# nanoporetech/bonito

Measured on AMD Instinct MI355X. Metric: signal samples/sec/GPU (chunk=10000, batch=512) + read accuracy vs ref, higher is better.
Workload: dtype f16

## Files before the change

bonito_amd/_lib.py:

```python
import ctypes as C
import os

_HERE = os.path.dirname(os.path.abspath(__file__))
LIB_PATH = os.environ.get("BONITO_HIP_LIB") or os.path.join(_HERE, "libbonito_hip.so")


class HipEngineError(RuntimeError):
    """An entry point of libbonito_hip.so reported an error."""


class bh_layer_t(C.Structure):
    _fields_ = [
        ("kind", C.c_int32), ("in_size", C.c_int32), ("out_size", C.c_int32),
        ("winlen", C.c_int32), ("stride", C.c_int32), ("padding", C.c_int32),
        ("activation", C.c_int32), ("reverse", C.c_int32),
        ("nhead", C.c_int32), ("dim_ff", C.c_int32), ("win_left", C.c_int32), ("win_right", C.c_int32),
        ("scale_factor", C.c_int32), ("groups", C.c_int32), ("add_residual", C.c_int32), ("quantize", C.c_int32), ("reserved_i", C.c_int32 * 1),
        ("scale", C.c_float), ("clamp_lo", C.c_float), ("clamp_hi", C.c_float),
        ("blank_score", C.c_float), ("alpha", C.c_float), ("eps", C.c_float), ("reserved_f", C.c_float * 2),
        ("w0", C.c_void_p), ("b0", C.c_void_p), ("w1", C.c_void_p), ("b1", C.c_void_p),
        ("w2", C.c_void_p), ("w3", C.c_void_p), ("w4", C.c_void_p), ("w5", C.c_void_p),
    ]


# ... 118 lines not shown
    "bh_host_map_finish": (_l, [_vp, _l, _vp, _l, _l, _vp, _l, _l, _vp, _l, _vp, _l, _vp, _l, _vp]),
    "bh_host_mean_qscore": (C.c_double, [C.c_char_p, _l]),
    "bh_host_svb16_decode": (_l, [_vp, _l, _l, _vp]),
    "bh_lstm_workspace": (_sz, [_i, _i]),
    "bh_lstm_layer": (_i, [_vp, _vp, _vp, _i, _i, _i, _i, _vp, _vp, _i, _vp]),
    "bh_lstm_q8_layer": (_i, [_vp, _f, _vp, _vp, _vp, _i, _i, _i, _i, _i, _vp, _vp, _vp, _vp]),
    "bh_lstm_q8_layer_split": (_i, [_vp, _f, _vp, _vp, _vp, _i, _i, _i, _i, _i, _vp, _vp, _vp, _i, _vp]),
    "bh_lstm_layer_family": (_i, [_vp, _vp, _vp, _vp, _i, _i, _i, _i, _i, _i, _vp, _vp]),
    "bh_lstm_launch_plan": (_i, [_i, _i, _i, _i, _i, C.POINTER(C.c_int32), _i]),
    "bh_optim_chunk": (_i, []),
    "bh_optim_workspace": (_sz, [_vp, _i]),
    "bh_optim_norm": (_i, [_vp, _vp, _i, _vp, _d, _i, _d, _d, _i, _d, _d, _vp, _sz, _vp]),
    "bh_optim_update": (_i, [_vp, _vp, _vp, _vp, _vp, _i, _vp, _d, _d, _d, _d, _d, _vp]),
    "bh_optim_last_kernel": (_i, []),
    "bh_encoder_debug_read": (_i, [_vp, _vp, _sz, _sz]),
    "bh_encoder_set_option": (_i, [_vp, C.c_char_p, _i]),
}

_lib = None


CONV_KERNELS = {"none": 0, "first": 1, "ws_384": 20, "ws_96": 21, "front3_384": 30, "front3_96": 31, "dwconv": 40, "igemm_base": 100}


def conv_igemm_code(ntt, fs):
    return CONV_KERNELS["igemm_base"] + 10 * ntt + int(fs)


CTC_LOSS_KERNELS = {1: 31, 2: 63, 4: 127, 8: 255, 104: 511, 108: 1023, 116: 2047}

# ... 44 lines not shown
```

bonito_amd/csrc/beam.hip:

```cpp
#include <stdlib.h>

#include "common.h"
#include "kernels.h"
#include "options.h"
#include <cstring>
#include "../../include/bh_lse_table.h"

namespace bh {

__device__ const float g_lse_tab[BH_LSE_TABLE_SIZE] = {BH_LSE_TABLE_VALUES};

__device__ __forceinline__ float lse2_tab(float a, float b, const float* tab) {
    float m = fmaxf(a, b);
    float d = fabsf(a - b);
    if (!(d < BH_LSE_RANGE)) return m;
    float x = d * BH_LSE_SCALE;
    int i = (int)x;
    float f = x - (float)i;
    float t0 = tab[i];
    float sp = __fmaf_rn(f, tab[i + 1] - t0, t0);
    return m + sp;
}

__device__ __forceinline__ float lse2_tab_nb(float a, float b, const float* tab) {
// ... 1126 lines not shown
    }
    if (DBG && lane == 0)
        for (int i = 0; i < 6; ++i) p.dbg[(long)n * 8 + i] = dsec[i];
}

struct FinArgs {
    const uint8_t* bp;
    const int* final_slot;
    const float* P;
    int N, T;
    float q_scale, q_offset;
    int8_t* sequence;
    int8_t* qstring;
    int8_t* moves;
    float* qfloat;
};

constexpr int FTB = 256;

__global__ __launch_bounds__(64) void beam_finalize_kernel(FinArgs p) {
    __shared__ __attribute__((aligned(16))) uint8_t st[FTB * MAXW];
    __shared__ int8_t res_m[FTB], res_s[FTB];
    __shared__ int s_r;
    const int n = blockIdx.x, lane = threadIdx.x;
    const int T = p.T;
    const uint8_t* bp = p.bp + (long)n * T * MAXW;
    const float* P = p.P + (long)n * T * 4;
    int8_t* sq = p.sequence + (long)n * T;
    int8_t* qs = p.qstring + (long)n * T;
    int8_t* mv = p.moves + (long)n * T;
    float* qf = p.qfloat ? p.qfloat + (long)n * T : nullptr;
    if (lane == 0) s_r = p.final_slot[n];
    for (int thi = T; thi > 0; thi -= FTB) {
        const int tlo = max(0, thi - FTB);
        const int nbytes = (thi - tlo) * MAXW;
        const uint4_t* src = (const uint4_t*)(bp + (long)tlo * MAXW);
        {
            constexpr int PER = FTB * MAXW / 16 / 64;
            uint4_t tmp[PER];
#pragma unroll
            for (int k = 0; k < PER; ++k)
                if (lane + 64 * k < nbytes / 16) tmp[k] = src[lane + 64 * k];
#pragma unroll
            for (int k = 0; k < PER; ++k)
                if (lane + 64 * k < nbytes / 16) ((uint4_t*)st)[lane + 64 * k] = tmp[k];
        }
        __syncthreads();
        if (lane == 0) {
            int r = s_r;
            for (int t = thi - 1; t >= tlo; --t) {
                const int info = st[(t - tlo) * MAXW + r];
                const int is_move = (info >> 5) & 1;
                res_m[t - tlo] = (int8_t)is_move;
                res_s[t - tlo] = is_move ? (int8_t)((0x54474341u >> (8 * (info >> 6))) & 0xffu) : (int8_t)0;
                r = info & 31;
            }
            s_r = r;
        }
        __syncthreads();
        for (int i = lane; i < thi - tlo; i += 64) {
            mv[tlo + i] = res_m[i];
            sq[tlo + i] = res_s[i];
            qs[tlo + i] = 0;
// ... 10 lines not shown
        const int c = sq[t];
        const int x = c == 'A' ? 0 : c == 'C' ? 1 : c == 'G' ? 2 : 3;
        double err = 0.0;
        for (int u = t; u < t2; ++u) {
            const float4_t pv = *(const float4_t*)(P + (long)u * 4);
#pragma unroll
            for (int y = 0; y < 4; ++y)
                if (y != x) err += (double)pv[y];
        }
        err /= (double)(t2 - t);
        if (err < 1e-10) err = 1e-10;
        float qv = (float)(-10.0 * log10(err)) * p.q_scale + p.q_offset;
        qv = fminf(fmaxf(qv, 1.0f), 50.0f);
        if (qf) qf[t] = qv;
        qs[t] = (int8_t)(33 + (int)floorf(qv + 0.5f));
    }
}

}

namespace {
using namespace bh;

size_t n_states(int state_len) {
    size_t S = 1;
    for (int i = 0; i < state_len; ++i) S *= 4;
    return S;
}

struct DecodeWorkspace {
// ... 183 lines not shown
    if (int rc = launch_instance(bs2_backward_instances, p.backward, stream, a2)) return rc;
    SideStream* side = p.forward_on_helper ? side_stream() : nullptr;
    if (side) {
        BH_CHECK_HIP(hipEventRecord(side->fork, stream));
        BH_CHECK_HIP(hipStreamWaitEvent(side->stream, side->fork, 0));
    }
    if (p.has_forward) {
        Bs2FwdArgs f2{(const half_t*)scores, beta, P, N, T, blank, p.nt};
        if (int rc = launch_instance(bs2_forward_instances, p.forward, side ? side->stream : stream, f2)) return rc;
    }
    if (side) BH_CHECK_HIP(hipEventRecord(side->join, side->stream));
    BeamArgs ba{(const half_t*)scores, beta, N, T, (int)n_states(state_len), state_len, beam_width, blank, logf(beam_cut), bp, fin,
                debug ? (long long*)(ws + w.dbg) : nullptr, p.select_radix ? 0.0f : 256.0f / fmaxf(logf(beam_cut), 1e-6f), P, p.nt};
    if (int rc = launch_instance(beam_instances, p.beam, stream, ba)) return rc;
    if (side) BH_CHECK_HIP(hipStreamWaitEvent(stream, side->join, 0));
    FinArgs fa{bp, fin, P, N, T, q_scale, q_offset, sequence, qstring, moves, qfloat};
    hipLaunchKernelGGL(beam_finalize_kernel, dim3(N), dim3(64), 0, stream, fa);
    BH_CHECK_HIP(hipGetLastError());
    return 0;
}

int bh_k_beam_search_plan(int N, int T, int state_len, int cu_count, int debug, int32_t* out, int n_out) {
    BH_REQUIRE(state_len >= 1 && state_len <= 5, "beam_search_plan: state_len must be in 1..5 (got %d)", state_len);
    BH_REQUIRE(N > 0 && T > 0 && out, "beam_search_plan: empty problem N=%d T=%d, or no record", N, T);
    const BeamPlan p = beam_plan(state_len, N, bh::g_opt, debug != 0, cu_count);
    const DecodeWorkspace w = decode_workspace(N, T, state_len);
    const int32_t plan[] = {bs2_backward_instances[p.backward.instance].key, p.backward.grid, p.backward.block, p.backward.lds,
                            p.has_forward, p.has_forward ? bs2_forward_instances[p.forward.instance].key : 0, p.forward.grid,
                            p.forward.block, p.forward.lds, p.forward_on_helper,
                            state_len, p.cpw, p.debug, p.fuse, p.beam.grid, p.beam.block, p.beam.lds, p.select_radix, p.nt};
    const size_t layout[] = {w.beta, w.Bcum, w.logZ, w.P, w.bp, w.fin, w.dbg, w.pv_bp, w.beam_total, w.pv_total};
    constexpr int n_plan = sizeof(plan) / sizeof(plan[0]), n_layout = sizeof(layout) / sizeof(layout[0]);
// ... 11 lines not shown
```

bonito_amd/csrc/engine.cpp:

```cpp
#include <hip/hip_runtime.h>
#include <stdarg.h>
#include <stdio.h>
#include <string.h>

#include <algorithm>
#include <atomic>
#include <cmath>
#include <string>
#include <vector>

#include "../../include/bonito_hip.h"
#include "common.h"
#include "devbuf.h"
#include "kernels.h"
#include "lstm_pack.h"
#include "options.h"

static thread_local char g_err[1024] = "";
void bh_set_error(const char* fmt, ...) {
    va_list ap;
    va_start(ap, fmt);
    vsnprintf(g_err, sizeof(g_err), fmt, ap);
    va_end(ap);
}
// ... 79 lines not shown
    std::vector<Layer> layers;
    DevBuf act[3], gates, sig, err, lstm_ws;
    static constexpr int ERR_SLOTS = 64;
    int* err_host = nullptr;
    std::atomic<long> ticket{-1};
    std::atomic<long> checked{-1};
    std::atomic<int> sticky{0};
    int* cur_err = nullptr;
    int n_act = 2;
    hipStream_t fill_stream = nullptr;
    hipEvent_t fill_ready = nullptr, fill_done = nullptr;
    void* prefilled = nullptr;
    int lstm_prefill = 1;
    DevBuf q_act[2], q_ex;
    DevBuf ex16;
    int lstm_pair = 1;
    int norm_fuse = 0;
    int lstm_exchange = 1;
    int lstm_q8 = 1;
    DevBuf res;
    DevBuf t_qkv, t_mid, t_a, t_b, rot;
    int rot_len = 0;
    int out_features = 0;
    int lstm_force_slow = 0, lstm_tune = 0;
    int batch_pad = 16;
    int lstm_wide = 1;
    int attn_ring = 1;
    int lstm_fused = 3;
    bool profiling = false;
    struct Span { int cls; hipEvent_t a, b; };
// ... 144 lines not shown
    if (!q8) {
        p.row = lstm_admits(d, p.family, wide && !ring ? BH_LSTM_V_OUTPUT : 0);
        p.geo = p.row->geo;
        p.handoff = p.geo.unlimited ? HANDOFF_LDS : p.row->ex_bytes ? HANDOFF_RING : HANDOFF_OUTPUT;
        if (!p.row->projects) {
            p.gate_w = l.lstm_ih[p.row->w_ih].p;
            p.gate_b = (const float*)(p.row->w_ih == BH_LSTM_W_WIDE_ROWS ? l.lstm_bias_wide : l.b0).p;
        }
    }
    p.n_rings = Np / p.geo.ring_chunks;
    p.rings_per_launch = p.geo.rings_per_launch(e->n_cus);
    p.pairs = p.family == BH_LSTM_WGX && e->lstm_pair;
    return p;
}

struct CreateState {
    int channels = 1, channels_eff = 1;
    float bound = 4.0f;
    bool any_q8 = false;
};

static int create_conv(bh_encoder* e, size_t i, const bh_layer_t& d, CreateState& cs) {
    Layer& L = e->layers[i];
    BH_REQUIRE(d.w0 && d.in_size > 0 && d.out_size > 0 && d.winlen > 0 && d.stride > 0, "encoder_create: layer %zu: malformed convolution", i);
    BH_REQUIRE(d.groups <= 1, "encoder_create: layer %zu: grouped conv not supported here", i);
    const bool next_is_conv = next_kind(e, i) == BH_LAYER_CONV;
    const int K = d.winlen;
    L.cin_eff = d.in_size == 1 ? 1 : cs.channels_eff;
    L.cout_eff = next_is_conv ? pad8(d.out_size) : d.out_size;
    BH_REQUIRE(d.in_size == 1 || (cs.channels == d.in_size && L.cin_eff >= d.in_size),
// ... 196 lines not shown
            bh_set_error("encoder_create: sentinel pre-fill resources");
            return -1;
        }
    }
    if (cs.any_q8) {
        if (e->q_act[0].alloc(ab + 256) || e->q_act[1].alloc(ab + 256) || e->q_ex.alloc((size_t)4 * (Np / 16) * 16 * 1024 + 256))
            return -1;
    }
    {
        size_t exb = 0;
        for (const auto& l : e->layers) {
            if (l.d.kind != BH_LAYER_LSTM) continue;
            for (const bh_lstm_instance* row : lstm_admitted(l.d)) exb = std::max(exb, (size_t)4 * (Np / row->geo.ring_chunks) * row->ex_bytes);
        }
        if (exb && e->ex16.alloc(exb + 256)) return -1;
    }
    if (e->act[0].alloc(ab + 256) || e->act[1].alloc(ab + 256) || e->gates.alloc(w.gate_bytes + 256) ||
        e->sig.alloc((size_t)Np * e->max_chunk * 2) || e->err.alloc(sizeof(int) * bh_encoder::ERR_SLOTS) ||
        e->lstm_ws.alloc(bh_k_lstm_ws_bytes(Np, 1024)))
        return -1;
    if (w.qkv_bytes) {
        if (e->t_qkv.alloc(w.qkv_bytes + 256) || e->t_mid.alloc(w.mid_bytes + 256) || e->t_a.alloc(w.model_bytes + 256) ||
            e->t_b.alloc(w.model_bytes + 256))
            return -1;
        std::vector<float> cs_table((size_t)w.max_tokens * 32 * 2);
        if (bh_rotary_table(w.max_tokens, 64, cs_table.data())) return -2;
        if (upload_f32(e->rot, cs_table.data(), cs_table.size())) return -1;
        e->rot_len = w.max_tokens;
    }
    if (hipHostMalloc((void**)&e->err_host, sizeof(int) * bh_encoder::ERR_SLOTS, hipHostMallocDefault) != hipSuccess) {
// ... 300 lines not shown
        }
    }
    e->prefilled = nullptr;
    if (next_kind(e, i) == BH_LAYER_LSTM) { rc = prefill_next(e, c, i, (size_t)M); if (rc) return rc; }
    ProfSpan span(e, st, BH_PROF_LSTM_REC);
    bh_lstm_launch layer{};
    layer.family = p.family;
    layer.input = p.gate_w ? e->gates.p : c.cur;
    layer.w_ih = l.lstm_ih[p.row->w_ih].p; layer.w_hh = l.lstm_hh[p.row->w_hh].p; layer.bias = (const float*)l.b0.p;
    layer.h_out = dst;
    layer.ex = p.handoff == HANDOFF_RING ? e->ex16.p : nullptr;
    layer.T = len; layer.N = Np; layer.H = H;
    layer.R = layer.n_rings = p.n_rings;
    layer.reverse = d.reverse;
    layer.err_flag = e->cur_err; layer.xcc_ws = (int*)e->lstm_ws.p;
    layer.write_through = e->lstm_force_slow; layer.tune = e->lstm_tune;
    rc = bh_k_lstm_run_layer(layer, p.rings_per_launch, p.pairs, st);
    if (rc) return rc;
    c.advance(dst); c.C = H;
    return 0;
}

static int forward_linear_crf(bh_encoder* e, size_t i, Cursor& c) {
    const Layer& l = e->layers[i];
    const bh_layer_t& d = l.d;
    BH_REQUIRE(c.lay == L_TNC || c.lay == L_NLC, "encoder_forward: linearcrfencoder needs encoded input");
    BH_REQUIRE(c.C == d.in_size, "encoder_forward: layer %zu expects %d features, got %d", i, d.in_size, c.C);
    const float sc = d.scale != 0.0f ? d.scale : 1.0f;
    int rc;
    ProfSpan span(e, c.st, BH_PROF_CRF_LINEAR);
// ... 144 lines not shown
    if (prev != e->device) BH_CHECK_HIP(hipSetDevice(e->device));
    struct Restore {
        int prev, dev;
        ~Restore() { if (prev != dev) (void)hipSetDevice(prev); }
    } restore{prev, e->device};

    {
        const long n = ++e->ticket;
        const int slot = (int)(n % bh_encoder::ERR_SLOTS);
        if (n - bh_encoder::ERR_SLOTS > e->checked.load()) e->sticky.fetch_or(((volatile int*)e->err_host)[slot]);
        ((volatile int*)e->err_host)[slot] = 0;
        e->cur_err = (int*)e->err.p + slot;
        BH_CHECK_HIP(hipMemsetAsync(e->cur_err, 0, sizeof(int), st));
    }
    const int Np = (N + e->batch_pad - 1) / e->batch_pad * e->batch_pad;
    if (Np != N) BH_CHECK_HIP(hipMemsetAsync((char*)e->sig.p + (size_t)N * L * 2, 0, (size_t)(Np - N) * L * 2, st));
    BH_CHECK_HIP(hipMemcpyAsync(e->sig.p, signal, (size_t)N * L * 2, hipMemcpyDeviceToDevice, st));

    e->prefilled = nullptr;
    Cursor c;
    c.cur = e->sig.p; c.len = L; c.N = N; c.Np = Np; c.st = st; c.scores = scores; c.n_act = e->n_act;
    for (size_t i = 0; i < e->layers.size(); ++i) {
        int rc = 0;
        switch (e->layers[i].d.kind) {
            case BH_LAYER_CLAMP: continue;
            case BH_LAYER_CONV: rc = forward_conv(e, i, c); break;
            case BH_LAYER_LSTM: rc = forward_lstm(e, i, c); break;
            case BH_LAYER_LINEAR_CRF: rc = forward_linear_crf(e, i, c); break;
            case BH_LAYER_LINEAR: rc = forward_linear(e, i, c); break;
            case BH_LAYER_TRANSFORMER: rc = forward_transformer(e, i, c); break;
            case BH_LAYER_DWCONV: rc = forward_dwconv(e, i, c); break;
            case BH_LAYER_RESIDUAL_PROJ: rc = forward_residual_proj(e, i, c); break;
            case BH_LAYER_CTC_DECODER: rc = forward_ctc_decoder(e, i, c); break;
            case BH_LAYER_UPSAMPLE: rc = forward_upsample(e, i, c); break;
            default: BH_REQUIRE(false, "encoder_forward: unsupported layer kind %d", e->layers[i].d.kind);
        }
// ... 69 lines not shown
        BH_CHECK_HIP(hipEventSynchronize(s.b));
        float t = 0.0f;
        BH_CHECK_HIP(hipEventElapsedTime(&t, s.a, s.b));
        if (s.cls >= 0 && s.cls < BH_PROF_CLASSES) { ms[s.cls] += t; launches[s.cls] += 1; }
        (void)hipEventDestroy(s.a); (void)hipEventDestroy(s.b);
    }
    e->spans.clear();
    return 0;
}

extern "C" int bh_encoder_debug_read(bh_encoder_t* e, void* host, size_t bytes, size_t offset) {
    BH_REQUIRE(e && host && offset + bytes <= e->lstm_ws.bytes, "encoder_debug_read: out of range");
    BH_CHECK_HIP(hipMemcpy(host, (char*)e->lstm_ws.p + offset, bytes, hipMemcpyDeviceToHost));
    return 0;
}
extern "C" int bh_encoder_set_option(bh_encoder_t* e, const char* name, int value) {
    BH_REQUIRE(e && name, "encoder_set_option: null argument");
    if (!strcmp(name, "lstm_force_slow")) { e->lstm_force_slow = value & 1; return 0; }
    if (!strcmp(name, "lstm_fused")) { e->lstm_fused = value; return 0; }
    if (!strcmp(name, "attn_ring")) { e->attn_ring = value; return 0; }
    if (!strcmp(name, "lstm_wide")) { e->lstm_wide = value; return 0; }
    if (!strcmp(name, "lstm_prefill")) { e->lstm_prefill = value; return 0; }
    if (!strcmp(name, "lstm_q8")) { e->lstm_q8 = value; return 0; }
    if (!strcmp(name, "lstm_exchange")) { e->lstm_exchange = value; return 0; }
    if (!strcmp(name, "lstm_pair")) { e->lstm_pair = value; return 0; }
    if (!strcmp(name, "norm_fuse")) { e->norm_fuse = value; return 0; }
    if (!strcmp(name, "gemm_v1")) { bh::g_opt.gemm_path = value; return 0; }
    if (!strcmp(name, "lstm_tune")) { e->lstm_tune = value; return 0; }
    BH_REQUIRE(false, "encoder_set_option: unknown option '%s'", name);
}
// ... 1 lines not shown
```

bonito_amd/csrc/kernels.h:

```cpp
#pragma once
#include <hip/hip_runtime.h>
#include <stdint.h>

#include "../../include/bonito_hip.h"

int bh_k_linear(const void* X, const void* W, const float* bias, void* out, int M, int N, int K,
                int ldx, int ldw, int ldo, int act, float scale, float clamp_lo, float clamp_hi,
                int gated, int row_div, long row_s_hi, long row_s_lo, int row_lim, hipStream_t stream,
                const void* residual = nullptr, int ldres = 0, float res_scale = 1.0f);
int bh_k_linear_last_kernel();

int bh_k_conv_first(const void* signal, const float* w, const float* bias, void* out, int N, int Lin,
                    int Lout, int Cout, int K, int stride, int pad, int act, float clamp_lo,
                    float clamp_hi, long os_n, long os_t, hipStream_t stream);
int bh_k_conv_igemm(const void* in, const void* wpk, const float* bias, void* out, int N, int Lin,
                    int Lout, int Cin, int Cout, int K, int stride, int pad, int act, float clamp_lo,
                    float clamp_hi, long os_n, long os_t, hipStream_t stream);
int bh_k_conv_last_kernel();
void bh_k_conv_note_kernel(int code);

struct bh_lstm_geometry {
    int ring_chunks = 16;
    int wgs_per_group = 0;
    int rings_per_slot = 1;
// ... 42 lines not shown
    bh_lstm_family family;
    const void* input;
    const void* w_ih;
    const void* w_hh;
    const float* bias;
    void* h_out;
    void* ex;
    int T, N, H;
    int R, n_rings;
    int reverse;
    int* err_flag;
    int* xcc_ws;
    int write_through;
    int tune;
    int arm;
};
int bh_k_lstm_launch(const bh_lstm_launch& l, hipStream_t stream);
int bh_k_lstm_run_layer(const bh_lstm_launch& layer, int rings_per_launch, bool pair, hipStream_t stream);
int bh_k_lstm_launch_plan(int family, int H, int flags, int n_rings, int cus, int32_t* out, int n_out);
size_t bh_k_lstm_ws_bytes(int N, int H);
int bh_k_fill_u16(void* dst, uint16_t value, size_t count, hipStream_t stream);

int bh_k_crf_viterbi(const void* scores, int N, int T, int state_len, int layout_5s, float blank_score,
                     long s_n, long s_t, void* bp_ws, float* alpha_ws, int8_t* moves, int8_t* path,
                     float* best_score, hipStream_t stream);

int bh_k_crf_revcomp(const void* in, void* out, int N, int T, int state_len, int layout_5s, long s_n, long s_t,
                     hipStream_t stream);

size_t bh_k_crf_seq_workspace(int N, int T, int Lmax, int state_len);
// ... 173 lines not shown
```

bonito_amd/csrc/lstm.hip:

```cpp
#include <string.h>
#include <type_traits>

#include "common.h"
#include "kernels.h"
#include "lstm_cell.h"
#include "lstm_ring.h"
#include "options.h"

namespace bh {

struct LstmArgs {
    const half_t* G;
    const half_t* whh;
    half_t* h;
    int T, N, H;
    int n_rings;
    int reverse;
    int* err;
    unsigned max_spins;
    int* xcc_ws;
    int force_slow;
    int tune;
};

// ... 1222 lines not shown
    p->grid = g.grid(n_rings);
    p->xcc_bytes = 0;
    p->arm_bytes = arm ? (size_t)4 * R * row->ex_bytes : 0;
    if (g.unlimited) return 0;
    BH_REQUIRE(g.wgs_per_group > 0 && p->grid <= g.resident(cus), "lstm: %d workgroups must be co-resident but the device has %d CUs; split the batch", p->grid, cus);
    p->xcc_bytes = (size_t)n_rings * row->slots_per_ring * sizeof(int);
    return 0;
}

int bh_k_lstm_launch(const bh_lstm_launch& l, hipStream_t stream) {
    using namespace bh;
    LstmLaunchPlan p;
    if (int rc = lstm_launch_plan(l.family, l.H, l.ex != nullptr, l.tune, l.N, l.R, l.n_rings, l.arm != 0, bh_cu_count(), &p)) return rc;
    const bh_lstm_instance& row = *p.row;
    BH_REQUIRE(!row.projects || l.input != l.h_out, "lstm: fused layer cannot run in place");
    if (!row.geo.unlimited) {
        BH_REQUIRE(l.xcc_ws != nullptr, "lstm: missing XCD agreement workspace");
        BH_CHECK_HIP(hipMemsetAsync(l.xcc_ws, 0xFF, p.xcc_bytes, stream));
    }
    if (p.arm_bytes) BH_CHECK_HIP(hipMemsetAsync(l.ex, 0xFF, p.arm_bytes, stream));
    const LstmArgs a{row.projects || row.args == ARGS_WIDE ? nullptr : (const half_t*)l.input, (const half_t*)l.w_hh, (half_t*)l.h_out,
                     l.T, l.N, l.H, l.n_rings, l.reverse, l.err_flag, max_spins(), l.xcc_ws, l.write_through, l.tune};
    const LstmFusedArgs fa{(const half_t*)l.input, (const half_t*)l.w_ih, l.bias, a};
    if (row.raise_lds) BH_CHECK_HIP(bh_max_lds(row.kernel, row.lds_bytes));
    const dim3 grid(p.grid), block(row.block);
    switch (row.args) {
        case ARGS_LSTM: hipLaunchKernelGGL(((void (*)(LstmArgs))row.kernel), grid, block, row.lds_bytes, stream, a); break;
        case ARGS_FUSED: hipLaunchKernelGGL(((void (*)(LstmFusedArgs))row.kernel), grid, block, row.lds_bytes, stream, fa); break;
        case ARGS_WGX:
            hipLaunchKernelGGL(((void (*)(LstmWgxArgs))row.kernel), grid, block, row.lds_bytes, stream, LstmWgxArgs{fa, (char*)l.ex, l.R});
            break;
        case ARGS_WIDE:
            hipLaunchKernelGGL(((void (*)(LstmWideArgs))row.kernel), grid, block, row.lds_bytes, stream,
                               LstmWideArgs{(const half_t*)l.input, a, (char*)l.ex, l.R});
            break;
// ... 4 lines not shown

int bh_k_lstm_run_layer(const bh_lstm_launch& layer, int rings_per_launch, bool pair, hipStream_t stream) {
    const bh_lstm_instance* row = bh_k_lstm_find(layer.family, layer.H, 0);
    BH_REQUIRE(row, "lstm: family %d has no instance for H=%d", layer.family, layer.H);
    BH_REQUIRE(rings_per_launch >= 1, "lstm: the device has too few CUs for hidden size %d", layer.H);
    for (int r0 = 0; r0 < layer.R;) {
        bh_lstm_launch l = layer;
        const bool pair_now = pair && layer.family == BH_LSTM_WGX && layer.R - r0 > rings_per_launch;
        if (pair_now) l.family = BH_LSTM_WGX2;
        l.n_rings = std::min(pair_now ? 2 * rings_per_launch : rings_per_launch, layer.R - r0);
        const size_t col = (size_t)r0 * row->geo.ring_chunks;
        l.input = (const char*)layer.input + col * (row->projects ? 1 : 4) * layer.H * 2;
        l.h_out = (char*)layer.h_out + col * layer.H * 2;
        if (layer.ex) l.ex = (char*)layer.ex + (size_t)r0 * row->ex_bytes;
        l.arm = r0 == 0;
        if (int rc = bh_k_lstm_launch(l, stream)) return rc;
        r0 += l.n_rings;
    }
    return 0;
}

int bh_k_lstm_launch_plan(int family, int H, int flags, int n_rings, int cus, int32_t* out, int n_out) {
    BH_REQUIRE(out && n_out >= BH_LSTM_PLAN_RECORD, "lstm_launch_plan: out must hold %d integers", (int)BH_LSTM_PLAN_RECORD);
    BH_REQUIRE(family >= BH_LSTM_WAVE && family <= BH_LSTM_Q8 && cus > 0, "lstm_launch_plan: family %d, %d CUs", family, cus);
    memset(out, 0, sizeof(int32_t) * BH_LSTM_PLAN_RECORD);
    if (family == BH_LSTM_Q8) return bh_k_lstm_q8_launch_plan(H, flags & 0xff, n_rings, cus, out);
    LstmLaunchPlan p{};
    const bh_lstm_instance* any = bh_k_lstm_find(family, H, 0);
    if (any) {
        const bh_lstm_geometry& g = any->geo;
// ... 13 lines not shown
```

bonito_amd/csrc/options.cpp:

```cpp
#include "options.h"

#include <string.h>

namespace bh {

Options g_opt;

#define BH_OPT(name) #name, &Options::name
static constexpr OptionRow OPTION_TABLE[] = {
    {BH_OPT(gemm_path), 0, Norm::keep, "linear GEMM kernel families: 0 auto, 1 = v1 only, 2 = no 256-tile kernel, 3 = no four-wave kernel, 5 = four-wave wherever legal"},
    {BH_OPT(gemm_tile16), 1, Norm::flag, "four-wave GEMM K-tile stream: 1 = 16x16x32 MFMAs, 0 = 32x32x16 (agree to fp16 rounding)"},
    {BH_OPT(gemm_order), 1, Norm::flag, "four-wave GEMM work order in an XCD: 1 = feature groups fastest, 0 = token blocks fastest (same bytes)"},
    {BH_OPT(gemm_gf), 0, Norm::keep, "four-wave GEMM feature tiles per block: 0 automatic, else rounded down to 1 / 2 / 4 / 8 / 16 / 32 (same bytes)"},
    {BH_OPT(gemm_stagger), 0, Norm::keep, "start-phase stagger of the persistent GEMM kernels, 0 = off (same bytes; measured without effect)"},
    {BH_OPT(attn_waves), 0, Norm::keep, "ring attention waves per workgroup: 0 automatic, 8, 12 (same results)"},
    {BH_OPT(attn_version), 2, Norm::one_or_two, "ring attention kernel: 2 = current, 1 = the first ring kernel"},
    {BH_OPT(attn_expt), 0, Norm::keep, "timing experiments of the ring attention kernel (bit mask): RESULTS ARE WRONG ON PURPOSE unless 0"},
    {BH_OPT(beam_fork), -1, Norm::keep, "posterior scan next to the beam kernel on a helper stream: -1 auto, 0 never, 1 always"},
    {BH_OPT(beam_select), 0, Norm::keep, "beam top-W selection: 0 histogram + boundary ranking, 1 radix search (same beams)"},
    {BH_OPT(beam_fuse), -1, Norm::keep, "forward / posterior scan as a second wave of the beam kernel: -1 auto (<= 256 states), 0 never, 1 always"},
    {BH_OPT(beam_cpw), 0, Norm::keep, "chunks per workgroup of the fused beam kernel at 256 states: 0 automatic, 1, 2, 4 (same bytes)"},
    {BH_OPT(decode_nt), 0, Norm::keep, "non-temporal score loads in the decode scans: 0 off"},
    {BH_OPT(viterbi_quad), 1, Norm::keep, "CRF Viterbi: 1 = four states per thread where the layout allows, 0 = the one-state kernel everywhere"},
    {BH_OPT(conv_ws), 1, Norm::keep, "weight-stationary kernel for the 384- / 96-channel 19-tap convolution: 1 on, 0 = generic implicit GEMM"},
    {BH_OPT(conv_fs), 1, Norm::keep, "feature-split instances of the implicit-GEMM convolution: 1 on, 0 = position-split"},
    {BH_OPT(conv_fuse), 1, Norm::keep, "conv1 -> conv2 -> conv3 as one kernel: 1 = 384-channel stacks, 2 = also 96-channel, 0 = three kernels"},
    {BH_OPT(conv_lds_kb), 64, Norm::positive_or_def, "KiB of LDS a workgroup of the implicit-GEMM convolution may take for its input span"},
    {BH_OPT(conv_front_pipe), 1, Norm::keep, "fused front end of the 384-channel stacks: 1 = conv1 / conv2 of the next block beside conv3 (12-wave pipeline), 0 = phase after phase (same bytes)"},
    {BH_OPT(conv_front_wgs), 0, Norm::keep, "workgroups of the pipelined front end: 0 = one per CU, n > 0 caps the grid (same bytes; test hook, A/B)"},
    {BH_OPT(lstm_max_spins), 1000000, Norm::nonneg_or_def, "bound of the recurrent kernels' exchange spin loops (0: the first incomplete poll round is a timeout)"},
    {BH_OPT(lstm_q8_variant), 0, Norm::keep, "geometry of the 8-bit recurrent kernel, read at bh_encoder_create: 0, 1, 2"},
};
#undef BH_OPT

static constexpr bool defaults_agree() {
    constexpr Options o{};
    for (const OptionRow& r : OPTION_TABLE)
        if (o.*r.member != r.def) return false;
    return true;
}
static_assert(defaults_agree(), "options.h and OPTION_TABLE state different defaults");
static_assert(sizeof(OPTION_TABLE) / sizeof(OPTION_TABLE[0]) == sizeof(Options) / sizeof(int), "every member of Options has exactly one row");

const OptionRow* find_option(const char* name) {
    for (const OptionRow& r : OPTION_TABLE)
        if (!strcmp(name, r.name)) return &r;
// ... 5 lines not shown
```

bonito_amd/csrc/options.h:

```cpp
#pragma once

namespace bh {

struct Options {
    int gemm_path = 0;
    int gemm_tile16 = 1;
    int gemm_order = 1;
    int gemm_gf = 0;
    int gemm_stagger = 0;
    int attn_waves = 0;
    int attn_version = 2;
    int attn_expt = 0;
    int beam_fork = -1;
    int beam_select = 0;
    int beam_fuse = -1;
    int beam_cpw = 0;
    int decode_nt = 0;
    int viterbi_quad = 1;
    int conv_ws = 1;
    int conv_fs = 1;
    int conv_fuse = 1;
    int conv_lds_kb = 64;
    int conv_front_pipe = 1;
    int conv_front_wgs = 0;
    int lstm_max_spins = 1000000;
    int lstm_q8_variant = 0;
};
extern Options g_opt;

enum class Norm {
    keep,
    flag,
    one_or_two,
    positive_or_def,
    nonneg_or_def
};
struct OptionRow {
    const char* name;
    int Options::*member;
    int def;
    Norm norm;
// ... 15 lines not shown
```

bonito_amd/decode.py:

```python
import ctypes as C

import numpy as np
import torch

from bonito_amd import _lib

_ALPHABET = np.frombuffer(b"NACGT", dtype=np.uint8)


def _check_scores(scores):
    if scores.dtype != torch.float16:
        raise TypeError("Expected fp16 but received %s" % scores.dtype)
    if not scores.is_cuda:
        raise _lib.HipEngineError("scores must live on a HIP device (no CPU decode fallback)")
    if not scores.is_contiguous():
        raise AssertionError("scores must be contiguous [N, T, C]")


def state_len_of(C_, n_base=4):
    sl, size = 0, n_base
    while size < C_:
        size *= n_base
        sl += 1
    if size != C_:
# ... 29 lines not shown
        def result(self):
            out = self.result_planes()
            return out[0], out[1], out[2]

    def submit(self, scores):
        _check_scores(scores)
        N, T, Cc = scores.shape
        if N > self.N or T != self.T or Cc != self.C:
            raise ValueError("decoder built for (<=%d, %d, %d), got %s" % (self.N, self.T, self.C, tuple(scores.shape)))
        lib = _lib.lib()
        bw, cut, blank, scale, offset = self.args
        out = self.dev_out
        with torch.cuda.device(self.device):
            st = _lib.stream_ptr(self.device)
            if self.mode == "beam":
                _lib.check(lib.bh_beam_search(_lib.ptr(scores), N, T, self.sl, bw, cut, blank, scale, offset,
                                              _lib.ptr(self.ws), _lib.ptr(out[0]), _lib.ptr(out[1]), _lib.ptr(out[2]),
                                              None, st), "bh_beam_search")
                for pl in range(3):
                    self.host_out[pl, :N].copy_(out[pl, :N], non_blocking=True)
            else:
                _lib.check(lib.bh_crf_viterbi(_lib.ptr(scores), N, T, self.sl, 0, blank, T * Cc, Cc, _lib.ptr(self.ws),
                                              _lib.ptr(out[2]), _lib.ptr(out[1]), None, st), "bh_crf_viterbi")
                for pl in (1, 2):
                    self.host_out[pl, :N].copy_(out[pl, :N], non_blocking=True)
            self.done.record(torch.cuda.current_stream(self.device))
        return CRFDecoder.Ticket(self, N)


def beam_search(scores, beam_width=32, beam_cut=100.0, scale=1.0, offset=0.0, blank_score=2.0, return_qfloat=False):
    _check_scores(scores)
    N, T, Cc = scores.shape
    sl = state_len_of(Cc)
    lib = _lib.lib()
    dev = scores.device
# ... 97 lines not shown
def posterior_viterbi(scores, blank_score=2.0):
    _check_scores(scores)
    N, T, Cc = scores.shape
    sl = state_len_of(Cc)
    lib = _lib.lib()
    dev = scores.device
    ws = torch.empty(lib.bh_crf_posterior_viterbi_workspace(N, T, sl), dtype=torch.uint8, device=dev)
    moves = torch.empty((N, T), dtype=torch.int8, device=dev)
    path = torch.empty((N, T), dtype=torch.int8, device=dev)
    with torch.cuda.device(dev):
        _lib.check(lib.bh_crf_posterior_viterbi(_lib.ptr(scores), N, T, sl, float(blank_score), _lib.ptr(ws),
                                                _lib.ptr(moves), _lib.ptr(path), _lib.stream_ptr(dev)), "bh_crf_posterior_viterbi")
    return moves.cpu(), path.cpu()


def set_option(name, value):
    _lib.check(_lib.lib().bh_set_option(name.encode(), int(value)), "bh_set_option")



def seq_layout(scores, state_len, blank_score=None):
    S = 4 ** int(state_len)
    if scores.dim() != 3 or scores.shape[-1] not in (4 * S, 5 * S):
        raise ValueError("scores of shape %s are neither [T, N, %d] nor [N, T, %d] (state_len %d)"
                         % (tuple(scores.shape), 5 * S, 4 * S, state_len))
    if scores.shape[-1] == 5 * S:
        T, N = scores.shape[:2]
        return N, T, 1, scores.stride(1), scores.stride(0)
    if blank_score is None:
        raise ValueError("koi-layout scores [N, T, %d] need blank_score" % (4 * S))
    N, T = scores.shape[:2]
    return N, T, 0, scores.stride(0), scores.stride(1)
# ... 335 lines not shown
```

include/bonito_hip.h:

```cpp
#ifndef BONITO_HIP_H
#define BONITO_HIP_H

#include <stddef.h>
#include <stdint.h>

#ifdef __cplusplus
extern "C" {
#endif

#define BH_ABI_VERSION 1

enum { BH_ACT_NONE = 0, BH_ACT_SWISH = 1, BH_ACT_TANH = 2, BH_ACT_RELU = 3 };

enum {
    BH_LAYER_CONV = 1,
    BH_LAYER_LSTM = 2,
    BH_LAYER_LINEAR_CRF = 3,
    BH_LAYER_CLAMP = 4,
    BH_LAYER_TRANSFORMER = 5,
    BH_LAYER_UPSAMPLE = 6,
    BH_LAYER_TCS_BLOCK = 7,
    BH_LAYER_CTC_DECODER = 8,
    BH_LAYER_DWCONV = 9,
    BH_LAYER_RESIDUAL_PROJ = 10,
// ... 32 lines not shown
typedef struct bh_encoder bh_encoder_t;

const char* bh_last_error(void);
int bh_abi_version(void);
size_t bh_sizeof_layer(void);
int bh_device_count(void);

int bh_encoder_create(const bh_layer_t* layers, int n_layers, int device, int max_batch, int max_chunk,
                      bh_encoder_t** out);
void bh_encoder_destroy(bh_encoder_t* enc);
int bh_encoder_output_shape(const bh_encoder_t* enc, int L, int* T, int* C, int* stride);
int bh_encoder_forward(bh_encoder_t* enc, const void* signal, int N, int L, void* scores, void* stream);
int bh_encoder_describe(const bh_encoder_t* enc, char* buf, size_t bytes);
int bh_encoder_set_option(bh_encoder_t* enc, const char* name, int value);
int bh_encoder_debug_read(bh_encoder_t* enc, void* host, size_t bytes, size_t offset);
int bh_encoder_check(bh_encoder_t* enc, void* stream);
int bh_encoder_error_flag(const bh_encoder_t* enc);
long bh_encoder_last_ticket(const bh_encoder_t* enc);
int bh_encoder_error_flag_at(const bh_encoder_t* enc, long ticket);
int bh_encoder_ack(bh_encoder_t* enc, long ticket);

enum { BH_PROF_CONV = 0, BH_PROF_LSTM_GEMM = 1, BH_PROF_FILL = 2, BH_PROF_LSTM_REC = 3, BH_PROF_CRF_LINEAR = 4,
       BH_PROF_ATTENTION = 5 , BH_PROF_MLP = 6 ,
       BH_PROF_OTHER = 7, BH_PROF_MLP_FC1 = 8 ,
       BH_PROF_ATTENTION_CORE = 9 , BH_PROF_CLASSES = 10 };
int bh_encoder_profile(bh_encoder_t* enc, int enable);
int bh_encoder_profile_read(bh_encoder_t* enc, float* ms , int* spans );

size_t bh_crf_viterbi_workspace(int N, int T, int state_len);
int bh_crf_viterbi(const void* scores, int N, int T, int state_len, int layout_5s, float blank_score,
// ... 268 lines not shown
```

Baseline: 446.7 million.

## Arm LSTM exchange once, read signal in place, parallel traceback, write beam output to host

Bundles four independent changes, all on by default. LSTM exchange and XCD-agreement regions are filled by one memset at the head of the forward instead of before every launch, and the first convolution reads the caller's signal directly when no padding is needed, skipping a staging copy. The beam finalize traceback composes per-segment back-pointer maps across all 64 lanes instead of one lane chasing pointers. The finalize kernel also writes sequence, qstring and moves straight into mapped host memory, removing separate device-to-host copies but relying on pinned-host pointer detection and extra workspace room.

```diff
diff --git a/bonito_amd/_lib.py b/bonito_amd/_lib.py
--- a/bonito_amd/_lib.py
+++ b/bonito_amd/_lib.py
@@ -156,6 +156,7 @@
     "bh_optim_update": (_i, [_vp, _vp, _vp, _vp, _vp, _i, _vp, _d, _d, _d, _d, _d, _vp]),
     "bh_optim_last_kernel": (_i, []),
     "bh_encoder_debug_read": (_i, [_vp, _vp, _sz, _sz]),
+    "bh_encoder_debug_read_signal": (_i, [_vp, _vp, _sz, _sz]),
     "bh_encoder_set_option": (_i, [_vp, C.c_char_p, _i]),
 }
 
diff --git a/bonito_amd/csrc/beam.hip b/bonito_amd/csrc/beam.hip
--- a/bonito_amd/csrc/beam.hip
+++ b/bonito_amd/csrc/beam.hip
@@ -1164,14 +1164,32 @@
     int8_t* qstring;
     int8_t* moves;
     float* qfloat;
+    int8_t* host_sequence;
+    int8_t* host_qstring;
+    int8_t* host_moves;
 };
 
+__device__ __forceinline__ void fin_row_to_host(int8_t* dst, const int8_t* src, int T, int lane) {
+    const int head = min(T, (int)((16 - ((uintptr_t)dst & 15)) & 15));
+    const int body = (T - head) / 16;
+    const int tail = head + body * 16;
+    if (lane < head) dst[lane] = src[lane];
+    for (int i = lane; i < body; i += 64) ((uint4_t*)(dst + head))[i] = ((const uint4_t*)(src + head))[i];
+    if (lane < T - tail) dst[tail + lane] = src[tail + lane];
+}
+
 constexpr int FTB = 256;
-
+constexpr int FSEG = FTB / 64;
+constexpr int FSEG_BYTES = FSEG * MAXW + 4;
+
+template <bool PAR>
 __global__ __launch_bounds__(64) void beam_finalize_kernel(FinArgs p) {
-    __shared__ __attribute__((aligned(16))) uint8_t st[FTB * MAXW];
+    __shared__ __attribute__((aligned(16))) uint8_t st[PAR ? 64 * FSEG_BYTES : FTB * MAXW];
+    __shared__ __attribute__((aligned(4))) uint8_t seg_map[PAR ? 64 * MAXW : 4];
+    __shared__ uint8_t seg_entry[64];
     __shared__ int8_t res_m[FTB], res_s[FTB];
     __shared__ int s_r;
+    static_assert(MAXW == 32 && FSEG * MAXW % 16 == 0, "beam_finalize_kernel: a segment is whole 16-byte pieces of 32-slot rows");
     const int n = blockIdx.x, lane = threadIdx.x;
     const int T = p.T;
     const uint8_t* bp = p.bp + (long)n * T * MAXW;
@@ -1193,10 +1211,60 @@
                 if (lane + 64 * k < nbytes / 16) tmp[k] = src[lane + 64 * k];
 #pragma unroll
             for (int k = 0; k < PER; ++k)
-                if (lane + 64 * k < nbytes / 16) ((uint4_t*)st)[lane + 64 * k] = tmp[k];
+                if (lane + 64 * k < nbytes / 16) {
+                    const int j = lane + 64 * k;
+                    if constexpr (PAR) {
+                        unsigned* d = (unsigned*)st + j * 4 + j / (FSEG * MAXW / 16);
+                        d[0] = tmp[k].x; d[1] = tmp[k].y; d[2] = tmp[k].z; d[3] = tmp[k].w;
+                    } else {
+                        ((uint4_t*)st)[j] = tmp[k];
+                    }
+                }
         }
         __syncthreads();
-        if (lane == 0) {
+        if constexpr (PAR) {
+            const int nrows = thi - tlo;
+            const int nseg = (nrows + FSEG - 1) / FSEG;
+            const int lo = lane * FSEG;
+            const int cnt = min(FSEG, nrows - lo);
+            const uint8_t* seg = st + lane * FSEG_BYTES;
+            if (lane < nseg) {
+                unsigned packed[MAXW / 4];
+#pragma unroll
+                for (int s = 0; s < MAXW; ++s) {
+                    int r = s;
+#pragma unroll
+                    for (int j = FSEG - 1; j >= 0; --j)
+                        if (j < cnt) r = seg[j * MAXW + r] & 31;
+                    if (s % 4 == 0) packed[s / 4] = (unsigned)r;
+                    else packed[s / 4] |= (unsigned)r << (8 * (s % 4));
+                }
+#pragma unroll
+                for (int w = 0; w < MAXW / 4; ++w) ((unsigned*)seg_map)[lane * (MAXW / 4) + w] = packed[w];
+            }
+            __syncthreads();
+            if (lane == 0) {
+                int r = s_r;
+                for (int l = nseg - 1; l >= 0; --l) {
+                    seg_entry[l] = (uint8_t)r;
+                    r = seg_map[l * MAXW + r];
+                }
+                s_r = r;
+            }
+            __syncthreads();
+            if (lane < nseg) {
+                int r = seg_entry[lane];
+#pragma unroll
+                for (int j = FSEG - 1; j >= 0; --j)
+                    if (j < cnt) {
+                        const int info = seg[j * MAXW + r];
+                        const int is_move = (info >> 5) & 1;
+                        res_m[lo + j] = (int8_t)is_move;
+                        res_s[lo + j] = is_move ? (int8_t)((0x54474341u >> (8 * (info >> 6))) & 0xffu) : (int8_t)0;
+                        r = info & 31;
+                    }
+            }
+        } else if (lane == 0) {
             int r = s_r;
             for (int t = thi - 1; t >= tlo; --t) {
                 const int info = st[(t - tlo) * MAXW + r];
@@ -1237,6 +1305,13 @@
         qv = fminf(fmaxf(qv, 1.0f), 50.0f);
         if (qf) qf[t] = qv;
         qs[t] = (int8_t)(33 + (int)floorf(qv + 0.5f));
+    }
+    if (p.host_sequence) {
+        __threadfence();
+        __syncthreads();
+        fin_row_to_host(p.host_sequence + (long)n * T, sq, T, lane);
+        fin_row_to_host(p.host_qstring + (long)n * T, qs, T, lane);
+        fin_row_to_host(p.host_moves + (long)n * T, mv, T, lane);
     }
 }
 
@@ -1450,8 +1525,31 @@
                 debug ? (long long*)(ws + w.dbg) : nullptr, p.select_radix ? 0.0f : 256.0f / fmaxf(logf(beam_cut), 1e-6f), P, p.nt};
     if (int rc = launch_instance(beam_instances, p.beam, stream, ba)) return rc;
     if (side) BH_CHECK_HIP(hipStreamWaitEvent(stream, side->join, 0));
-    FinArgs fa{bp, fin, P, N, T, q_scale, q_offset, sequence, qstring, moves, qfloat};
-    hipLaunchKernelGGL(beam_finalize_kernel, dim3(N), dim3(64), 0, stream, fa);
+    FinArgs fa{bp, fin, P, N, T, q_scale, q_offset, sequence, qstring, moves, qfloat, nullptr, nullptr, nullptr};
+    if (bh::g_opt.beam_out_host) {
+        int8_t* out[3] = {sequence, qstring, moves};
+        int8_t* mapped[3] = {nullptr, nullptr, nullptr};
+        int n_host = 0;
+        for (int i = 0; i < 3; ++i) {
+            hipPointerAttribute_t at{};
+            if (hipPointerGetAttributes(&at, out[i]) != hipSuccess) { (void)hipGetLastError(); continue; }
+            if (at.type != hipMemoryTypeHost || !at.devicePointer) continue;
+            mapped[i] = (int8_t*)at.devicePointer;
+            ++n_host;
+        }
+        BH_REQUIRE(n_host == 0 || n_host == 3, "beam_search: sequence, qstring and moves must all be device memory or all be host memory");
+        if (n_host == 3) {
+            const size_t plane = ((size_t)N * T + 15) / 16 * 16 + 16;
+            BH_REQUIRE(3 * plane <= w.P - w.Bcum, "beam_search: no room for the device copies of host output planes");
+            BH_REQUIRE(((uintptr_t)(ws + w.Bcum) & 15) == 0, "beam_search: workspace must be 16-byte aligned for host output planes");
+            int8_t* dev[3];
+            for (int i = 0; i < 3; ++i) dev[i] = (int8_t*)(ws + w.Bcum) + i * plane + ((uintptr_t)mapped[i] & 15);
+            fa.sequence = dev[0]; fa.qstring = dev[1]; fa.moves = dev[2];
+            fa.host_sequence = mapped[0]; fa.host_qstring = mapped[1]; fa.host_moves = mapped[2];
+        }
+    }
+    if (bh::g_opt.fin_parallel) hipLaunchKernelGGL(beam_finalize_kernel<true>, dim3(N), dim3(64), 0, stream, fa);
+    else hipLaunchKernelGGL(beam_finalize_kernel<false>, dim3(N), dim3(64), 0, stream, fa);
     BH_CHECK_HIP(hipGetLastError());
     return 0;
 }
diff --git a/bonito_amd/csrc/engine.cpp b/bonito_amd/csrc/engine.cpp
--- a/bonito_amd/csrc/engine.cpp
+++ b/bonito_amd/csrc/engine.cpp
@@ -117,6 +117,8 @@
     int lstm_prefill = 1;
     DevBuf q_act[2], q_ex;
     DevBuf ex16;
+    DevBuf arm_ws;
+    std::vector<size_t> arm_off;
     int lstm_pair = 1;
     int norm_fuse = 0;
     int lstm_exchange = 1;
@@ -291,6 +293,19 @@
     return p;
 }
 
+constexpr size_t NO_ARM_REGION = ~(size_t)0;
+struct ArmRegion {
+    size_t ex_bytes = 0, xcc_bytes = 0;
+    size_t bytes() const { return (ex_bytes + xcc_bytes + 255) & ~(size_t)255; }
+};
+static ArmRegion arm_region(const LstmPlan& p) {
+    ArmRegion r;
+    if (p.family == BH_LSTM_Q8 || !p.row || p.geo.unlimited) return r;
+    if (p.handoff == HANDOFF_RING) r.ex_bytes = (size_t)4 * p.n_rings * p.row->ex_bytes;
+    r.xcc_bytes = (size_t)p.n_rings * p.row->slots_per_ring * sizeof(int);
+    return r;
+}
+
 struct CreateState {
     int channels = 1, channels_eff = 1;
     float bound = 4.0f;
@@ -517,6 +532,19 @@
             for (const bh_lstm_instance* row : lstm_admitted(l.d)) exb = std::max(exb, (size_t)4 * (Np / row->geo.ring_chunks) * row->ex_bytes);
         }
         if (exb && e->ex16.alloc(exb + 256)) return -1;
+        size_t armb = 0;
+        for (const auto& l : e->layers) {
+            if (l.d.kind != BH_LAYER_LSTM) continue;
+            ArmRegion r;
+            for (const bh_lstm_instance* row : lstm_admitted(l.d)) {
+                const size_t R = Np / row->geo.ring_chunks;
+                r.ex_bytes = std::max(r.ex_bytes, 4 * R * row->ex_bytes);
+                r.xcc_bytes = std::max(r.xcc_bytes, R * row->slots_per_ring * sizeof(int));
+            }
+            armb += r.bytes();
+        }
+        if (armb && e->arm_ws.alloc(armb)) return -1;
+        e->arm_off.assign(n_layers, NO_ARM_REGION);
     }
     if (e->act[0].alloc(ab + 256) || e->act[1].alloc(ab + 256) || e->gates.alloc(w.gate_bytes + 256) ||
         e->sig.alloc((size_t)Np * e->max_chunk * 2) || e->err.alloc(sizeof(int) * bh_encoder::ERR_SLOTS) ||
@@ -847,6 +875,13 @@
     layer.R = layer.n_rings = p.n_rings;
     layer.reverse = d.reverse;
     layer.err_flag = e->cur_err; layer.xcc_ws = (int*)e->lstm_ws.p;
+    if (e->arm_off[i] != NO_ARM_REGION) {
+        char* region = (char*)e->arm_ws.p + e->arm_off[i];
+        const ArmRegion r = arm_region(p);
+        if (r.ex_bytes) layer.ex = region;
+        layer.xcc_ws = (int*)(region + r.ex_bytes);
+        layer.armed = 1;
+    }
     layer.write_through = e->lstm_force_slow; layer.tune = e->lstm_tune;
     rc = bh_k_lstm_run_layer(layer, p.rings_per_launch, p.pairs, st);
     if (rc) return rc;
@@ -1021,12 +1056,28 @@
         BH_CHECK_HIP(hipMemsetAsync(e->cur_err, 0, sizeof(int), st));
     }
     const int Np = (N + e->batch_pad - 1) / e->batch_pad * e->batch_pad;
-    if (Np != N) BH_CHECK_HIP(hipMemsetAsync((char*)e->sig.p + (size_t)N * L * 2, 0, (size_t)(Np - N) * L * 2, st));
-    BH_CHECK_HIP(hipMemcpyAsync(e->sig.p, signal, (size_t)N * L * 2, hipMemcpyDeviceToDevice, st));
+    {
+        size_t arm_bytes = 0;
+        const bool arm_once = bh::g_opt.lstm_arm_once && e->arm_ws.p && !(e->lstm_tune & 4);
+        for (size_t i = 0; i < e->layers.size(); ++i) {
+            e->arm_off[i] = NO_ARM_REGION;
+            if (!arm_once || e->layers[i].d.kind != BH_LAYER_LSTM) continue;
+            const size_t b = arm_region(lstm_plan(e, e->layers[i], Np)).bytes();
+            if (!b || arm_bytes + b > e->arm_ws.bytes) continue;
+            e->arm_off[i] = arm_bytes;
+            arm_bytes += b;
+        }
+        if (arm_bytes) BH_CHECK_HIP(hipMemsetAsync(e->arm_ws.p, 0xFF, arm_bytes, st));
+    }
+    const bool direct = bh::g_opt.sig_direct && Np == N && ((uintptr_t)signal & 15) == 0 && e->layers[0].d.kind == BH_LAYER_CONV;
+    if (!direct) {
+        if (Np != N) BH_CHECK_HIP(hipMemsetAsync((char*)e->sig.p + (size_t)N * L * 2, 0, (size_t)(Np - N) * L * 2, st));
+        BH_CHECK_HIP(hipMemcpyAsync(e->sig.p, signal, (size_t)N * L * 2, hipMemcpyDeviceToDevice, st));
+    }
 
     e->prefilled = nullptr;
     Cursor c;
-    c.cur = e->sig.p; c.len = L; c.N = N; c.Np = Np; c.st = st; c.scores = scores; c.n_act = e->n_act;
+    c.cur = direct ? signal : e->sig.p; c.len = L; c.N = N; c.Np = Np; c.st = st; c.scores = scores; c.n_act = e->n_act;
     for (size_t i = 0; i < e->layers.size(); ++i) {
         int rc = 0;
         switch (e->layers[i].d.kind) {
@@ -1126,6 +1177,11 @@
     BH_CHECK_HIP(hipMemcpy(host, (char*)e->lstm_ws.p + offset, bytes, hipMemcpyDeviceToHost));
     return 0;
 }
+extern "C" int bh_encoder_debug_read_signal(bh_encoder_t* e, void* host, size_t bytes, size_t offset) {
+    BH_REQUIRE(e && host && offset + bytes <= e->sig.bytes, "encoder_debug_read_signal: out of range");
+    BH_CHECK_HIP(hipMemcpy(host, (char*)e->sig.p + offset, bytes, hipMemcpyDeviceToHost));
+    return 0;
+}
 extern "C" int bh_encoder_set_option(bh_encoder_t* e, const char* name, int value) {
     BH_REQUIRE(e && name, "encoder_set_option: null argument");
     if (!strcmp(name, "lstm_force_slow")) { e->lstm_force_slow = value & 1; return 0; }
diff --git a/bonito_amd/csrc/kernels.h b/bonito_amd/csrc/kernels.h
--- a/bonito_amd/csrc/kernels.h
+++ b/bonito_amd/csrc/kernels.h
@@ -80,6 +80,7 @@
     int write_through;
     int tune;
     int arm;
+    int armed;
 };
 int bh_k_lstm_launch(const bh_lstm_launch& l, hipStream_t stream);
 int bh_k_lstm_run_layer(const bh_lstm_launch& layer, int rings_per_launch, bool pair, hipStream_t stream);
diff --git a/bonito_amd/csrc/lstm.hip b/bonito_amd/csrc/lstm.hip
--- a/bonito_amd/csrc/lstm.hip
+++ b/bonito_amd/csrc/lstm.hip
@@ -1260,11 +1260,11 @@
     if (int rc = lstm_launch_plan(l.family, l.H, l.ex != nullptr, l.tune, l.N, l.R, l.n_rings, l.arm != 0, bh_cu_count(), &p)) return rc;
     const bh_lstm_instance& row = *p.row;
     BH_REQUIRE(!row.projects || l.input != l.h_out, "lstm: fused layer cannot run in place");
-    if (!row.geo.unlimited) {
-        BH_REQUIRE(l.xcc_ws != nullptr, "lstm: missing XCD agreement workspace");
-        BH_CHECK_HIP(hipMemsetAsync(l.xcc_ws, 0xFF, p.xcc_bytes, stream));
-    }
-    if (p.arm_bytes) BH_CHECK_HIP(hipMemsetAsync(l.ex, 0xFF, p.arm_bytes, stream));
+    if (!row.geo.unlimited) BH_REQUIRE(l.xcc_ws != nullptr, "lstm: missing XCD agreement workspace");
+    if (!l.armed) {
+        if (!row.geo.unlimited) BH_CHECK_HIP(hipMemsetAsync(l.xcc_ws, 0xFF, p.xcc_bytes, stream));
+        if (p.arm_bytes) BH_CHECK_HIP(hipMemsetAsync(l.ex, 0xFF, p.arm_bytes, stream));
+    }
     const LstmArgs a{row.projects || row.args == ARGS_WIDE ? nullptr : (const half_t*)l.input, (const half_t*)l.w_hh, (half_t*)l.h_out,
                      l.T, l.N, l.H, l.n_rings, l.reverse, l.err_flag, max_spins(), l.xcc_ws, l.write_through, l.tune};
     const LstmFusedArgs fa{(const half_t*)l.input, (const half_t*)l.w_ih, l.bias, a};
@@ -1299,6 +1299,7 @@
         l.h_out = (char*)layer.h_out + col * layer.H * 2;
         if (layer.ex) l.ex = (char*)layer.ex + (size_t)r0 * row->ex_bytes;
         l.arm = r0 == 0;
+        if (layer.armed && layer.xcc_ws) l.xcc_ws = layer.xcc_ws + (size_t)r0 * row->slots_per_ring;
         if (int rc = bh_k_lstm_launch(l, stream)) return rc;
         r0 += l.n_rings;
     }
diff --git a/bonito_amd/csrc/options.cpp b/bonito_amd/csrc/options.cpp
--- a/bonito_amd/csrc/options.cpp
+++ b/bonito_amd/csrc/options.cpp
@@ -30,6 +30,10 @@
     {BH_OPT(conv_front_wgs), 0, Norm::keep, "workgroups of the pipelined front end: 0 = one per CU, n > 0 caps the grid (same bytes; test hook, A/B)"},
     {BH_OPT(lstm_max_spins), 1000000, Norm::nonneg_or_def, "bound of the recurrent kernels' exchange spin loops (0: the first incomplete poll round is a timeout)"},
     {BH_OPT(lstm_q8_variant), 0, Norm::keep, "geometry of the 8-bit recurrent kernel, read at bh_encoder_create: 0, 1, 2"},
+    {BH_OPT(lstm_arm_once), 1, Norm::flag, "engine forward: 1 = every recurrent launch has its own exchange region, all armed by one fill at the head of the forward, 0 = fills in front of every launch (same bytes)"},
+    {BH_OPT(sig_direct), 1, Norm::flag, "engine forward: 1 = the first convolution reads the caller's signal in place where no padding row is needed, 0 = always staged (same bytes)"},
+    {BH_OPT(beam_out_host), 1, Norm::flag, "beam search: 1 = output planes in host memory are written row by row by the finalize kernel, 0 = every output pointer is handed to the kernels as it is"},
+    {BH_OPT(fin_parallel), 1, Norm::flag, "beam finalize traceback: 1 = composed back-pointer maps on all lanes, 0 = one lane chases the pointers (same bytes)"},
 };
 #undef BH_OPT
 
diff --git a/bonito_amd/csrc/options.h b/bonito_amd/csrc/options.h
--- a/bonito_amd/csrc/options.h
+++ b/bonito_amd/csrc/options.h
@@ -25,6 +25,10 @@
     int conv_front_wgs = 0;
     int lstm_max_spins = 1000000;
     int lstm_q8_variant = 0;
+    int lstm_arm_once = 1;
+    int sig_direct = 1;
+    int beam_out_host = 1;
+    int fin_parallel = 1;
 };
 extern Options g_opt;
 
diff --git a/bonito_amd/decode.py b/bonito_amd/decode.py
--- a/bonito_amd/decode.py
+++ b/bonito_amd/decode.py
@@ -67,11 +67,15 @@
         with torch.cuda.device(self.device):
             st = _lib.stream_ptr(self.device)
             if self.mode == "beam":
+                host = _OPTIONS.get("beam_out_host", 1) != 0
+                if host:
+                    out = self.host_out
                 _lib.check(lib.bh_beam_search(_lib.ptr(scores), N, T, self.sl, bw, cut, blank, scale, offset,
                                               _lib.ptr(self.ws), _lib.ptr(out[0]), _lib.ptr(out[1]), _lib.ptr(out[2]),
                                               None, st), "bh_beam_search")
-                for pl in range(3):
-                    self.host_out[pl, :N].copy_(out[pl, :N], non_blocking=True)
+                if not host:
+                    for pl in range(3):
+                        self.host_out[pl, :N].copy_(out[pl, :N], non_blocking=True)
             else:
                 _lib.check(lib.bh_crf_viterbi(_lib.ptr(scores), N, T, self.sl, 0, blank, T * Cc, Cc, _lib.ptr(self.ws),
                                               _lib.ptr(out[2]), _lib.ptr(out[1]), None, st), "bh_crf_viterbi")
@@ -199,8 +203,12 @@
     return moves.cpu(), path.cpu()
 
 
+_OPTIONS = {}
+
+
 def set_option(name, value):
     _lib.check(_lib.lib().bh_set_option(name.encode(), int(value)), "bh_set_option")
+    _OPTIONS[name] = int(value)
 
 
 
diff --git a/include/bonito_hip.h b/include/bonito_hip.h
--- a/include/bonito_hip.h
+++ b/include/bonito_hip.h
@@ -70,6 +70,7 @@
 int bh_encoder_describe(const bh_encoder_t* enc, char* buf, size_t bytes);
 int bh_encoder_set_option(bh_encoder_t* enc, const char* name, int value);
 int bh_encoder_debug_read(bh_encoder_t* enc, void* host, size_t bytes, size_t offset);
+int bh_encoder_debug_read_signal(bh_encoder_t* enc, void* host, size_t bytes, size_t offset);
 int bh_encoder_check(bh_encoder_t* enc, void* stream);
 int bh_encoder_error_flag(const bh_encoder_t* enc);
 long bh_encoder_last_ticket(const bh_encoder_t* enc);
```

Result: no change. 444.4 million (-0.5%).
